# 1pathplanningzzj/pointnet_refine

Hardware: AMD Instinct MI355X
Metric: lane segments/sec (fwd+bwd) at B=4096,N=1024; HBM GB/s vs roofline (higher is better)
Workload: dtype f32 (large GEMMs: 2xfp16-split MFMA, 3 products, fp32 accumulate); 1 GPU; LineRefineNet training step (fwd + deep-supervision L1 + bwd + Adam), B=4096/GPU, N=1024, M=32, C=4; global_batch=4096, points=1024, parallelism=dp1, decoder_chunk=4096

## Files before the change

include/pointnet_refine_hip.h:

```cpp
#ifndef POINTNET_REFINE_HIP_H
#define POINTNET_REFINE_HIP_H

#include <stddef.h>
#include <stdint.h>

#ifdef __cplusplus
extern "C" {
#endif

#define PRH_OK 0
#define PRH_ERR_ARG (-1)
#define PRH_ERR_WORKSPACE (-2)
#define PRH_ERR_HIP (-3)

#define PRH_MAX_LAYERS 8

typedef struct {
  const float* w;
  const float* b;
  const float* gamma;
  const float* beta;
  float* running_mean;
  float* running_var;
  int64_t* num_batches_tracked;
// ... 17 lines not shown
  const float* gate_w2;
  const float* gate_b2;
} prh_encoder_params;

typedef struct {
  prh_bn_layer_grad conv[5];
  prh_bn_layer_grad fusion;
  float* d_gate_w1; float* d_gate_b1; float* d_gate_w2; float* d_gate_b2;
} prh_encoder_grads;

typedef struct {
  float* z_cat;
  float* z_fus;
  float* gate;
  float* bn_scale;
  float* bn_shift;
  float* bn_mean;
  float* bn_rstd;
  int32_t* argmax;
  float* op_amax;
} prh_encoder_saved;

size_t prh_encoder_workspace_bytes(int B, int N, int in_channel, int out_dim, int backward);

int prh_encoder_forward(const prh_encoder_params* prm, const float* ctx, int B, int N,
                        int training, float momentum, float eps,
                        float* fused, float* gfeat, const prh_encoder_saved* saved,
                        void* workspace, size_t workspace_bytes, int device, void* stream);

int prh_encoder_backward(const prh_encoder_params* prm, const float* ctx, int B, int N,
                         int training, float* d_fused, const float* d_gfeat, int d_fused_scratch,
                         const prh_encoder_saved* saved, const prh_encoder_grads* grads,
                         float* d_ctx, void* workspace, size_t workspace_bytes, int device,
                         void* stream);

typedef struct {
  uint16_t* z_cat;
  uint16_t* z_fus;
  uint16_t* gate;
  float* bn_scale;
  float* bn_shift;
  float* bn_mean;
  float* bn_rstd;
  int32_t* argmax;
} prh_encoder_saved_bf16;
size_t prh_encoder_bf16_workspace_bytes(int B, int N, int in_channel, int out_dim, int backward);
// ... 178 lines not shown
```

pointnet_refine_amd/_lib.py:

```python
from __future__ import annotations

import ctypes as C
import os
import subprocess
import threading

_HERE = os.path.dirname(os.path.abspath(__file__))
_ROOT = os.path.dirname(_HERE)
LIB_PATH = os.environ.get("PRH_LIB_PATH") or os.path.join(_HERE, "libpointnet_refine_hip.so")
_CSRC = os.path.join(_HERE, "csrc")
_SOURCES = [os.path.join(_CSRC, "prh_lib.hip")] + (sorted(
    os.path.join(_CSRC, f) for f in os.listdir(_CSRC) if f.endswith((".hpp", ".h", ".hip")) and f != "prh_lib.hip")
    if os.path.isdir(_CSRC) else [])
_HEADER = os.path.join(_ROOT, "include", "pointnet_refine_hip.h")

PRH_MAX_LAYERS = 8


class BnLayer(C.Structure):
    _fields_ = [("w", C.c_void_p), ("b", C.c_void_p), ("gamma", C.c_void_p), ("beta", C.c_void_p),
                ("running_mean", C.c_void_p), ("running_var", C.c_void_p),
                ("num_batches_tracked", C.c_void_p), ("cin", C.c_int), ("cout", C.c_int)]


# ... 5 lines not shown
    _fields_ = [("in_channel", C.c_int), ("out_dim", C.c_int), ("conv", BnLayer * 5),
                ("fusion", BnLayer), ("gate_w1", C.c_void_p), ("gate_b1", C.c_void_p),
                ("gate_w2", C.c_void_p), ("gate_b2", C.c_void_p)]


class EncoderGrads(C.Structure):
    _fields_ = [("conv", BnLayerGrad * 5), ("fusion", BnLayerGrad), ("d_gate_w1", C.c_void_p),
                ("d_gate_b1", C.c_void_p), ("d_gate_w2", C.c_void_p), ("d_gate_b2", C.c_void_p)]


class EncoderSaved(C.Structure):
    _fields_ = [("z_cat", C.c_void_p), ("z_fus", C.c_void_p), ("gate", C.c_void_p),
                ("bn_scale", C.c_void_p), ("bn_shift", C.c_void_p), ("bn_mean", C.c_void_p),
                ("bn_rstd", C.c_void_p), ("argmax", C.c_void_p), ("op_amax", C.c_void_p)]


class EncoderSavedBf16(C.Structure):
    _fields_ = [("z_cat", C.c_void_p), ("z_fus", C.c_void_p), ("gate", C.c_void_p),
                ("bn_scale", C.c_void_p), ("bn_shift", C.c_void_p), ("bn_mean", C.c_void_p),
                ("bn_rstd", C.c_void_p), ("argmax", C.c_void_p)]


EXPORTS = [
    "prh_encoder_workspace_bytes", "prh_encoder_forward", "prh_encoder_backward",
    "prh_encoder_bf16_workspace_bytes", "prh_encoder_forward_bf16", "prh_encoder_backward_bf16",
    "prh_linear_bf16_workspace_bytes", "prh_linear_forward_bf16", "prh_linear_backward_bf16",
    "prh_linear_forward_out16", "prh_linear_backward_dy16", "prh_attn_forward_kv16", "prh_attn_backward_kv16",
    "prh_encoder_fused_image_bytes", "prh_encoder_fused_prepare", "prh_encoder_fused_workspace_bytes",
    "prh_encoder_fused_forward",
    "prh_linear_forward_workspace_bytes", "prh_linear_forward", "prh_linear_forward_ex",
    "prh_linear_forward_full", "prh_operand_absmax_workspace_bytes", "prh_operand_absmax",
    "prh_linear_uses_operand_maxima", "prh_linear_backward_full", "prh_pos_hidden_forward", "prh_pos_hidden_backward_workspace_bytes",
    "prh_pos_hidden_backward", "prh_linear_small_forward", "prh_linear_small_backward_workspace_bytes",
    "prh_linear_small_backward",
    "prh_linear_backward_workspace_bytes", "prh_linear_backward", "prh_linear_backward_ex",
    "prh_mlp_stack_workspace_bytes", "prh_mlp_stack_forward", "prh_mlp_stack_backward",
    "prh_test_gemm_nt", "prh_test_gemm_tn_workspace_bytes", "prh_test_gemm_tn", "prh_test_xcc_map",
    "prh_profile_enable", "prh_profile_count", "prh_profile_reset", "prh_profile_read",
    "prh_attn_forward", "prh_attn_backward", "prh_attn_backward_ex",
    "prh_context_workspace_bytes", "prh_context_build",
    "prh_line_metrics", "prh_shift_sweep_workspace_bytes", "prh_shift_sweep",
    "prh_l1_loss_workspace_bytes", "prh_l1_loss", "prh_adam_step",
    "prh_add_dropout_layernorm_forward", "prh_add_dropout_layernorm_workspace_bytes",
    "prh_add_dropout_layernorm_backward",
    "prh_relu_mask_absmax", "prh_cast_perm_bf16", "prh_posmem_images", "prh_attn_fold_forward", "prh_set_gemm_mode", "prh_get_gemm_mode", "prh_set_dropout_seed_source",
    "prh_last_error", "prh_version",
]
# ... 7 lines not shown
        return True
    t = os.path.getmtime(LIB_PATH)
    return any(os.path.exists(s) and os.path.getmtime(s) > t for s in _SOURCES + [_HEADER])


def build(force: bool = False, verbose: bool = False) -> str:
    if not force and not needs_build():
        return LIB_PATH
    hipcc = os.environ.get("HIPCC", "/opt/rocm/bin/hipcc")
    cmd = [hipcc, "--offload-arch=gfx950", "-O3", "-std=c++17", "-shared", "-fPIC",
           "-o", LIB_PATH, _SOURCES[0]]
    if verbose:
        print(" ".join(cmd))
    subprocess.run(cmd, check=True)
    return LIB_PATH


def _bind(lib):
    vp, i, f, sz, lg = C.c_void_p, C.c_int, C.c_float, C.c_size_t, C.c_long
    lib.prh_last_error.restype = C.c_char_p
    lib.prh_version.restype = C.c_char_p
    lib.prh_encoder_workspace_bytes.restype = sz
    lib.prh_encoder_workspace_bytes.argtypes = [i, i, i, i, i]
    lib.prh_encoder_forward.restype = i
    lib.prh_encoder_forward.argtypes = [C.POINTER(EncoderParams), vp, i, i, i, f, f, vp, vp,
                                        C.POINTER(EncoderSaved), vp, sz, i, vp]
    lib.prh_encoder_backward.restype = i
    lib.prh_encoder_backward.argtypes = [C.POINTER(EncoderParams), vp, i, i, i, vp, vp, i,
                                         C.POINTER(EncoderSaved), C.POINTER(EncoderGrads), vp, vp,
                                         sz, i, vp]
    lib.prh_encoder_bf16_workspace_bytes.restype = sz
    lib.prh_encoder_bf16_workspace_bytes.argtypes = [i, i, i, i, i]
    lib.prh_encoder_forward_bf16.restype = i
    lib.prh_encoder_forward_bf16.argtypes = [C.POINTER(EncoderParams), vp, i, i, i, f, f, vp, vp,
                                             C.POINTER(EncoderSavedBf16), vp, sz, i, vp]
    lib.prh_encoder_backward_bf16.restype = i
    lib.prh_encoder_backward_bf16.argtypes = [C.POINTER(EncoderParams), vp, i, i, i, vp, vp,
                                              C.POINTER(EncoderSavedBf16), C.POINTER(EncoderGrads), vp, vp,
                                              sz, i, vp]
    lib.prh_linear_bf16_workspace_bytes.restype = sz
    lib.prh_linear_bf16_workspace_bytes.argtypes = [i, i, i, i]
    lib.prh_linear_forward_bf16.restype = i
    lib.prh_linear_forward_bf16.argtypes = [vp, lg, vp, vp, vp, i, i, i, i, vp, sz, i, vp]
    lib.prh_linear_backward_bf16.restype = i
    lib.prh_linear_backward_bf16.argtypes = [vp, lg, vp, vp, vp, vp, vp, i, i, i, vp, sz, i, vp]
    lib.prh_linear_forward_out16.restype = i
# ... 141 lines not shown
```

pointnet_refine_amd/csrc/prh_gemm.hpp:

```cpp
#pragma once
#include <hip/hip_runtime.h>
#include <type_traits>
#include <stdint.h>

namespace prh {

typedef float f32x16 __attribute__((ext_vector_type(16)));

enum { PRO_NONE = 0, PRO_BNRELU = 1, PRO_BNBWD = 2, PRO_GATE1 = 3 };
enum { EPI_BIAS = 0, EPI_BIAS_STATS = 1, EPI_GATE = 2, EPI_DGRAD = 3 };

enum {
  F_RELU_OUT = 1,
  F_ACCUM = 2,
  F_MASK = 4,
  F_STATS = 8,
  F_STORE_GATE = 16,
  F_E1_ROWVEC = 32,
  F_RESID = 64,
  F_DROPOUT = 256,
  F_POOL = 128,
};

struct NTParams {
// ... 41 lines not shown

__device__ __forceinline__ int lds_off(int row, int slot) {
  return row * BK + ((slot ^ ((row >> 1) & 7)) << 2);
}

template <int PRO>
__device__ __forceinline__ float4 pro_apply(float4 a, float4 a2, float4 ka, float4 kb, float4 kc) {
  float4 o;
  if (PRO == PRO_NONE) {
    o = a;
  } else if (PRO == PRO_BNRELU) {
    o.x = fmaxf(fmaf(a.x, ka.x, kb.x), 0.f); o.y = fmaxf(fmaf(a.y, ka.y, kb.y), 0.f);
    o.z = fmaxf(fmaf(a.z, ka.z, kb.z), 0.f); o.w = fmaxf(fmaf(a.w, ka.w, kb.w), 0.f);
  } else if (PRO == PRO_BNBWD) {
    o.x = fmaf(ka.x, a.x, fmaf(kb.x, a2.x, kc.x)); o.y = fmaf(ka.y, a.y, fmaf(kb.y, a2.y, kc.y));
    o.z = fmaf(ka.z, a.z, fmaf(kb.z, a2.z, kc.z)); o.w = fmaf(ka.w, a.w, fmaf(kb.w, a2.w, kc.w));
  } else {
    o.x = fmaxf(fmaf(a.x, ka.x, kb.x), 0.f); o.y = fmaxf(fmaf(a.x, ka.y, kb.y), 0.f);
    o.z = fmaxf(fmaf(a.x, ka.z, kb.z), 0.f); o.w = fmaxf(fmaf(a.x, ka.w, kb.w), 0.f);
  }
  return o;
}

__device__ __forceinline__ float4 ldg4(const float* p) { return *reinterpret_cast<const float4*>(p); }
__device__ __forceinline__ float4 zero4() { return make_float4(0.f, 0.f, 0.f, 0.f); }

template <int EPI, int MT, int NT>
__device__ __forceinline__ void nt_epilogue(f32x16 (&acc)[MT][NT], const NTParams& p, int rbase_,
                                            int cbase, int rb, int lane) {
  const int half = lane >> 5, l31 = lane & 31;
  const int rbase = __builtin_amdgcn_readfirstlane(rbase_);
  float* __restrict__ Cb = p.C + (size_t)rbase * p.ldc;
  const float* __restrict__ Eb = p.E1 != nullptr ? p.E1 + (size_t)rbase * p.lde1 : nullptr;
  float* __restrict__ C2b = p.C2 != nullptr ? p.C2 + (size_t)rbase * p.ldc2 : nullptr;
  const int ldc = (int)p.ldc, lde1 = (int)p.lde1, ldc2 = (int)p.ldc2;
  const int mrows = p.M - rbase;
  const unsigned dseed = (EPI == EPI_BIAS && (p.flags & F_DROPOUT) != 0) ? epi_seed(p) : 0u;
#pragma unroll
  for (int nt = 0; nt < NT; ++nt) {
    const int col = cbase + nt * 32 + l31;
    const bool cok = col < p.N;
    const float bias = (p.bias != nullptr && cok) ? p.bias[col] : 0.f;

    if (EPI == EPI_BIAS || EPI == EPI_BIAS_STATS) {
      float s = 0.f;
#pragma unroll
// ... 34 lines not shown
          float mx = -3.0e38f, mn = 3.0e38f;
#pragma unroll
          for (int mt = 0; mt < MT; ++mt)
#pragma unroll
            for (int r = 0; r < 16; ++r)
              if (mt * 32 + crow(r, half) < mrows) { mx = fmaxf(mx, acc[mt][nt][r]); mn = fminf(mn, acc[mt][nt][r]); }
          mx = fmaxf(mx, __shfl_xor(mx, 32));
          mn = fminf(mn, __shfl_xor(mn, 32));
          if (half == 0 && cok) {
            p.ws_c[(size_t)rb * p.N + col] = mx;
            p.ws_d[(size_t)rb * p.N + col] = mn;
          }
        }
      }
    } else if (EPI == EPI_GATE) {
      const float es = cok ? p.es[col] : 0.f, et = cok ? p.et[col] : 0.f;
#pragma unroll
      for (int mt = 0; mt < MT; ++mt)
#pragma unroll
        for (int r = 0; r < 16; ++r) {
          const int lr = mt * 32 + crow(r, half);
          if (lr < mrows && cok) {
            const float g = acc[mt][nt][r] + bias;
            const float m = 0.5f + 0.5f / (1.f + __expf(-g));
            const float zf = Eb[lr * lde1 + col];
            const float rl = fmaxf(fmaf(zf, es, et), 0.f);
            Cb[lr * ldc + col] = rl * m;
            if ((p.flags & F_STORE_GATE) != 0) C2b[lr * ldc2 + col] = m;
          }
        }
    } else {
      const bool mask = (p.flags & F_MASK) != 0, accum = (p.flags & F_ACCUM) != 0;
      const bool need_z = mask || (p.flags & F_STATS) != 0;
      const int ecol = (p.flags & F_E1_ROWVEC) ? 0 : col;
      const float es = (mask && cok) ? p.es[col] : 0.f, et = (mask && cok) ? p.et[col] : 0.f;
      float s1 = 0.f, s2 = 0.f;
#pragma unroll
      for (int mt = 0; mt < MT; ++mt)
#pragma unroll
        for (int r = 0; r < 16; ++r) {
          const int lr = mt * 32 + crow(r, half);
          if (lr < mrows && cok) {
            float v = acc[mt][nt][r] + bias;
            if (accum) v += Cb[lr * ldc + col];
            float z = 0.f;
            if (need_z) z = Eb[lr * lde1 + ecol];
            if (mask && !(fmaf(z, es, et) > 0.f)) v = 0.f;
// ... 261 lines not shown
      const int lr = mt * 32 + lrow;
      const bool ok = lr < mrows && c4ok;
      float4 v = *reinterpret_cast<const float4*>(scratch + lrow * EPI_LDW + c4);
      v.x += bias4.x; v.y += bias4.y; v.z += bias4.z; v.w += bias4.w;
      const float4 z = zz[b & 1][i];
      const float4 o = oo[b & 1][i];
      if (EPI == EPI_DGRAD) {
        v.x += o.x; v.y += o.y; v.z += o.z; v.w += o.w;
        if (mask) {
          v.x = fmaf(z.x, es4.x, et4.x) > 0.f ? v.x : 0.f;
          v.y = fmaf(z.y, es4.y, et4.y) > 0.f ? v.y : 0.f;
          v.z = fmaf(z.z, es4.z, et4.z) > 0.f ? v.z : 0.f;
          v.w = fmaf(z.w, es4.w, et4.w) > 0.f ? v.w : 0.f;
        }
        if (C16) {
          v.x = bf16_round(v.x); v.y = bf16_round(v.y); v.z = bf16_round(v.z); v.w = bf16_round(v.w);
        }
        const float4 q = ok ? v : zero4();
        s1.x += q.x; s1.y += q.y; s1.z += q.z; s1.w += q.w;
        s2.x = fmaf(q.x, z.x, s2.x); s2.y = fmaf(q.y, z.y, s2.y);
        s2.z = fmaf(q.z, z.z, s2.z); s2.w = fmaf(q.w, z.w, s2.w);
      } else if (EPI == EPI_GATE) {
        float4 m;
        m.x = 0.5f + 0.5f / (1.f + __expf(-v.x)); m.y = 0.5f + 0.5f / (1.f + __expf(-v.y));
        m.z = 0.5f + 0.5f / (1.f + __expf(-v.z)); m.w = 0.5f + 0.5f / (1.f + __expf(-v.w));
        v.x = fmaxf(fmaf(z.x, es4.x, et4.x), 0.f) * m.x; v.y = fmaxf(fmaf(z.y, es4.y, et4.y), 0.f) * m.y;
        v.z = fmaxf(fmaf(z.z, es4.z, et4.z), 0.f) * m.z; v.w = fmaxf(fmaf(z.w, es4.w, et4.w), 0.f) * m.w;
        if (ok && (p.flags & F_STORE_GATE) != 0) st4e<C16>(C2b, lr * ldc2 + col4, m);
        if (pool && ok) {
          if (C16) { v.x = bf16_round(v.x); v.y = bf16_round(v.y); v.z = bf16_round(v.z); v.w = bf16_round(v.w); }
          const float vv[4] = {v.x, v.y, v.z, v.w};
#pragma unroll
          for (int e = 0; e < 4; ++e) {
            if (vv[e] > pmx[e]) { pmx[e] = vv[e]; pix[e] = lr; }
            psm[e] += vv[e];
          }
        }
      } else {
        if (resid) { v.x += z.x; v.y += z.y; v.z += z.z; v.w += z.w; }
        if ((p.flags & F_RELU_OUT) != 0) {
          v.x = fmaxf(v.x, 0.f); v.y = fmaxf(v.y, 0.f); v.z = fmaxf(v.z, 0.f); v.w = fmaxf(v.w, 0.f);
        }
        if (EPI == EPI_BIAS && (p.flags & F_DROPOUT) != 0) {
          const unsigned rw = (unsigned)(rbase + lr), c0 = (unsigned)col4;
          v.x = epi_keep(dseed, rw, c0, p.drop_thresh) ? v.x * p.drop_scale : 0.f;
          v.y = epi_keep(dseed, rw, c0 + 1, p.drop_thresh) ? v.y * p.drop_scale : 0.f;
          v.z = epi_keep(dseed, rw, c0 + 2, p.drop_thresh) ? v.z * p.drop_scale : 0.f;
          v.w = epi_keep(dseed, rw, c0 + 3, p.drop_thresh) ? v.w * p.drop_scale : 0.f;
// ... 147 lines not shown
      if (it == 0) epi_block_to_scratch(acc, mt, scratch, lane);
      const int lrow = it * 4 + rr;
      const int lr = mt * 32 + lrow;
      const bool ok = lr < mrows && c4ok;
      float4 v = *reinterpret_cast<const float4*>(scratch + lrow * EPI_LDW + c4);
      v.x += bias4.x; v.y += bias4.y; v.z += bias4.z; v.w += bias4.w;
      const float4 z = ev_f4(zz[b & 1][i]);
      const float4 o = ev_f4(oo[b & 1][i]);
      if (EPI == EPI_DGRAD) {
        v.x += o.x; v.y += o.y; v.z += o.z; v.w += o.w;
        v.x = fmaf(z.x, es4.x, et4.x) > mthr ? v.x : 0.f;
        v.y = fmaf(z.y, es4.y, et4.y) > mthr ? v.y : 0.f;
        v.z = fmaf(z.z, es4.z, et4.z) > mthr ? v.z : 0.f;
        v.w = fmaf(z.w, es4.w, et4.w) > mthr ? v.w : 0.f;
        if (C16) {
          v.x = bf16_round(v.x); v.y = bf16_round(v.y); v.z = bf16_round(v.z); v.w = bf16_round(v.w);
        }
        const float4 q = ok ? v : zero4();
        s1.x += q.x; s1.y += q.y; s1.z += q.z; s1.w += q.w;
        s2.x = fmaf(q.x, z.x, s2.x); s2.y = fmaf(q.y, z.y, s2.y);
        s2.z = fmaf(q.z, z.z, s2.z); s2.w = fmaf(q.w, z.w, s2.w);
      } else if (EPI == EPI_GATE) {
        float4 m;
        m.x = 0.5f + 0.5f / (1.f + __expf(-v.x)); m.y = 0.5f + 0.5f / (1.f + __expf(-v.y));
        m.z = 0.5f + 0.5f / (1.f + __expf(-v.z)); m.w = 0.5f + 0.5f / (1.f + __expf(-v.w));
        v.x = fmaxf(fmaf(z.x, es4.x, et4.x), 0.f) * m.x; v.y = fmaxf(fmaf(z.y, es4.y, et4.y), 0.f) * m.y;
        v.z = fmaxf(fmaf(z.z, es4.z, et4.z), 0.f) * m.z; v.w = fmaxf(fmaf(z.w, es4.w, et4.w), 0.f) * m.w;
        if ((p.flags & F_STORE_GATE) != 0) ev_store(rsC2, lr * rowC2 + vC, m);
        if (pool && ok) {
          if (C16) { v.x = bf16_round(v.x); v.y = bf16_round(v.y); v.z = bf16_round(v.z); v.w = bf16_round(v.w); }
          const float vv[4] = {v.x, v.y, v.z, v.w};
#pragma unroll
          for (int e = 0; e < 4; ++e) {
            if (vv[e] > pmx[e]) { pmx[e] = vv[e]; pix[e] = lr; }
            psm[e] += vv[e];
          }
        }
      } else {
        if (resid) { v.x += z.x; v.y += z.y; v.z += z.z; v.w += z.w; }
        if ((p.flags & F_RELU_OUT) != 0) {
          v.x = fmaxf(v.x, 0.f); v.y = fmaxf(v.y, 0.f); v.z = fmaxf(v.z, 0.f); v.w = fmaxf(v.w, 0.f);
        }
        if (EPI == EPI_BIAS && (p.flags & F_DROPOUT) != 0) {
          const unsigned rw = (unsigned)(rbase + lr), c0 = (unsigned)col4;
          v.x = epi_keep(dseed, rw, c0, p.drop_thresh) ? v.x * p.drop_scale : 0.f;
          v.y = epi_keep(dseed, rw, c0 + 1, p.drop_thresh) ? v.y * p.drop_scale : 0.f;
          v.z = epi_keep(dseed, rw, c0 + 2, p.drop_thresh) ? v.z * p.drop_scale : 0.f;
          v.w = epi_keep(dseed, rw, c0 + 3, p.drop_thresh) ? v.w * p.drop_scale : 0.f;
// ... 282 lines not shown
```

pointnet_refine_amd/csrc/prh_gemm_h2.hpp:

```cpp
#pragma once
#include "prh_gemm_s3.hpp"

namespace prh {

constexpr int H2_BK = 32;
constexpr int H2_PLANE = 256 * H2_BK * 2;
constexpr int H2_OPER = 2 * H2_PLANE;
constexpr int H2_STAGE = 2 * H2_OPER;
constexpr int H2_LDS = 2 * H2_STAGE;

__device__ __forceinline__ int h2_off(int row, int k) {
  return row * 64 + ((((k >> 3) ^ (-(row >> 2))) & 3) << 4) + ((k & 7) << 1);
}

inline size_t h2_weight_bytes(int N, int K) {
  return S3_WHDR + (size_t)((N + 255) / 256) * ((K + H2_BK - 1) / H2_BK) * H2_OPER;
}

__global__ __launch_bounds__(256) void prep_weights_h2_kernel(const float* __restrict__ W, int N,
                                                              int K, long ldw, char* __restrict__ out,
                                                              const float* __restrict__ amax) {
  const int KT = (K + H2_BK - 1) / H2_BK;
  const int NT_ = (N + 255) / 256;
  const long total = (long)NT_ * 256 * KT * 4;
// ... 2 lines not shown
  const int chunk = (int)(i & 3);
  long t = i >> 2;
  const int k_tile = (int)(t % KT); t /= KT;
  const int row = (int)(t & 255);
  const int n_tile = (int)(t >> 8);
  const int n = n_tile * 256 + row;
  const float S = pow2_scale(load_amax(amax));
  float v[8];
#pragma unroll
  for (int j = 0; j < 8; ++j) {
    const int k = k_tile * H2_BK + chunk * 8 + j;
    v[j] = (n < N && k < K) ? W[(size_t)n * ldw + k] * S : 0.f;
  }
  uint4 h, l;
  split2h(v[0], v[1], h.x, l.x);
  split2h(v[2], v[3], h.y, l.y);
  split2h(v[4], v[5], h.z, l.z);
  split2h(v[6], v[7], h.w, l.w);
  char* base = out + ((size_t)n_tile * KT + k_tile) * H2_OPER + h2_off(row, chunk * 8);
  *reinterpret_cast<uint4*>(base) = h;
  *reinterpret_cast<uint4*>(base + H2_PLANE) = l;
}

template <int I0 = 0, int I1 = 8>
__device__ __forceinline__ void h2_compute(f32x4 (&acc)[8][4], const char* st, int wm, int wn, int l15,
                                           int kc) {
  f16x8 wh[4], wl[4];
#pragma unroll
  for (int j = 0; j < 4; ++j) {
    const char* q = st + H2_OPER + h2_off(wn + j * 16 + l15, kc * 8);
    wh[j] = *reinterpret_cast<const f16x8*>(q);
    wl[j] = *reinterpret_cast<const f16x8*>(q + H2_PLANE);
  }
#pragma unroll
  for (int i = I0; i < I1; ++i) {
    const char* q = st + h2_off(wm + i * 16 + l15, kc * 8);
    const f16x8 ah = *reinterpret_cast<const f16x8*>(q);
    const f16x8 al = *reinterpret_cast<const f16x8*>(q + H2_PLANE);
#pragma unroll
    for (int j = 0; j < 4; ++j) {
      acc[i][j] = __builtin_amdgcn_mfma_f32_16x16x32_f16(al, wh[j], acc[i][j], 0, 0, 0);
      acc[i][j] = __builtin_amdgcn_mfma_f32_16x16x32_f16(ah, wl[j], acc[i][j], 0, 0, 0);
      acc[i][j] = __builtin_amdgcn_mfma_f32_16x16x32_f16(ah, wh[j], acc[i][j], 0, 0, 0);
    }
  }
}

template <int PRO, int EPI, bool PP = false>
__global__ __launch_bounds__(512, 2) void gemm_nt_h2_kernel(const NTParams p,
                                                            const char* __restrict__ Wp) {
  static_assert(PRO == PRO_NONE || PRO == PRO_BNRELU || PRO == PRO_GATE1, "prologue not supported");
  extern __shared__ __attribute__((aligned(16))) char smem[];
#ifdef PRH_STAMP
  unsigned t_acc[4] = {0u, 0u, 0u, 0u};
  unsigned long long t_prev = __builtin_amdgcn_s_memtime();
#endif
  const int tid = threadIdx.x, lane = tid & 63, wave = tid >> 6;
  const int l15 = lane & 15, kc = lane >> 4;
  const int wm = (wave >> 2) * 128, wn = (wave & 3) * 64;
  const int vb = xcd_remap(blockIdx.x, gridDim.x);
  const int tile_n = vb % p.tiles_n, tile_m = vb / p.tiles_n;
  const int m0 = tile_m * 256, n0 = tile_n * 256;
  const int KT = (p.K + H2_BK - 1) / H2_BK;

  const int sc = (tid & 7) * 4;
  const int sr = tid >> 3;
  const int KP = (KT + 2) * H2_BK;
// ... 438 lines not shown
```

pointnet_refine_amd/csrc/prh_lib.hip:

```cpp
#include "../../include/pointnet_refine_hip.h"

#include <hip/hip_runtime.h>
#include <stdarg.h>
#include <stdio.h>
#include <string.h>

#include <mutex>
#include <vector>

#include <stdlib.h>

#include "prh_gemm.hpp"
#include "prh_attn.hpp"
#include "prh_attn16.hpp"
#include "prh_gemm_s3.hpp"
#include "prh_gemm_h2.hpp"
#include "prh_b16.hpp"
#include "prh_small.hpp"
#include "prh_attnfold.hpp"
#include "prh_fused.hpp"
#include "prh_context.hpp"
#include "prh_metrics.hpp"
#include "prh_kernels.hpp"

// ... 1281 lines not shown
  LAUNCH_CHECK();
  StatInfo si; si.count = cdiv(P, 64); si.rows = 64;
  return stack_backward(c, layers, L, x, P, training, dy_cat, ldz, z_cat, ldz, bn_scale, bn_shift,
                        bn_mean, bn_rstd, grads, dx, w, sc, si, st);
}

static int enc_cat(const prh_encoder_params* prm) {
  int c = 0;
  for (int l = 0; l < 5; ++l) c += prm->conv[l].cout;
  return c;
}

size_t prh_encoder_workspace_bytes(int B, int N, int in_channel, int out_dim, int backward) {
  const int P = B * N;
  prh_bn_layer ly[5];
  const int ch[6] = {in_channel, 64, 128, 256, 512, out_dim};
  for (int l = 0; l < 5; ++l) { ly[l].cin = ch[l]; ly[l].cout = ch[l + 1]; }
  const int cat = 64 + 128 + 256 + 512 + out_dim;
  Arena a; EncWS e;
  enc_carve(cores_of(gemm_mode()), a, e, P, ly, cat, out_dim, backward);
  return a.off + 256;
}

static int check_encoder(const prh_encoder_params* prm) {
  if (!prm) return fail(PRH_ERR_ARG, "encoder: null params");
  if (prm->in_channel < 4) return fail(PRH_ERR_ARG, "encoder: expected input to have at least 4 channels (x,y,z,intensity), got %d", prm->in_channel);
  if (prm->conv[0].cin != prm->in_channel) return fail(PRH_ERR_ARG, "encoder: conv1.cin != in_channel");
  TRY(check_stack(prm->conv, 5));
  if (prm->conv[4].cout != prm->out_dim) return fail(PRH_ERR_ARG, "encoder: conv5.cout != out_dim");
  if (prm->fusion.cin != enc_cat(prm) || prm->fusion.cout != prm->out_dim)
    return fail(PRH_ERR_ARG, "encoder: fusion layer shape mismatch");
  if (prm->out_dim % 4) return fail(PRH_ERR_ARG, "encoder: out_dim must be a multiple of 4");
  if (!prm->fusion.w || !prm->fusion.b || !prm->fusion.gamma || !prm->fusion.beta ||
      !prm->fusion.running_mean || !prm->fusion.running_var || !prm->gate_w1 || !prm->gate_b1 ||
      !prm->gate_w2 || !prm->gate_b2)
    return fail(PRH_ERR_ARG, "encoder: null parameter pointer");
  return PRH_OK;
}

int prh_encoder_forward(const prh_encoder_params* prm, const float* ctx, int B, int N,
                        int training, float momentum, float eps, float* fused, float* gfeat,
                        const prh_encoder_saved* sv, void* workspace, size_t workspace_bytes,
                        int device, void* stream) {
  TRY(check_encoder(prm));
  if (!ctx || !fused || !sv || !sv->z_cat || !sv->z_fus || !sv->bn_scale || !sv->bn_shift ||
      !sv->bn_mean || !sv->bn_rstd || B <= 0 || N <= 0)
// ... 18 lines not shown
    NTParams p; memset(&p, 0, sizeof(p));
    p.A = sv->z_cat; p.lda = cat; p.W = prm->fusion.w; p.ldw = cat; p.K = cat;
    p.pa = sv->bn_scale; p.pb = sv->bn_shift;
    p.M = P; p.N = od; p.bias = prm->fusion.b; p.C = sv->z_fus; p.ldc = od;
    p.ws_a = w.ws_a; p.ws_b = w.ws_b; p.wprep = w.wprep;
    if (op_amax != nullptr) {
      hipLaunchKernelGGL(max_of_kernel, dim3(1), dim3(1), 0, st, (const float*)op_amax, 5, op_amax + 5);
      LAUNCH_CHECK();
      p.amaxA = op_amax + 5;
      p.ws_c = w.ws_c; p.ws_d = w.ws_d;
    }
    StatInfo si;
    if (training) TRY((launch_nt<PRO_BNRELU, EPI_BIAS_STATS>(c, p, st, &si)));
    else TRY((launch_nt<PRO_BNRELU, EPI_BIAS>(c, p, st)));
    TRY(bn_coeffs(prm->fusion, P, training, momentum, eps, w.ws_a, w.ws_b, w.stat2, si, sv->bn_mean + cat,
                  sv->bn_rstd + cat, sv->bn_scale + cat, sv->bn_shift + cat, st, w.ws_c, w.ws_d, w.apart,
                  op_amax ? op_amax + 6 : nullptr));
  }
  {
    NTParams p; memset(&p, 0, sizeof(p));
    p.A = ctx + 3; p.lda = C; p.pa = prm->gate_w1; p.pb = prm->gate_b1;
    p.W = prm->gate_w2; p.ldw = 64; p.K = 64; p.M = P; p.N = od; p.bias = prm->gate_b2;
    p.E1 = sv->z_fus; p.lde1 = od; p.es = sv->bn_scale + cat; p.et = sv->bn_shift + cat;
    p.C = fused; p.ldc = od; p.C2 = sv->gate; p.ldc2 = od;
    p.wprep = w.wprep;
    p.flags = sv->gate ? F_STORE_GATE : 0;
    const bool fuse_pool = gfeat != nullptr && (N % 128) == 0 && c.mode == 3 &&
                           nt_use_s3(c, P, od, 64) && (od & 3) == 0;
    if (fuse_pool) { p.flags |= F_POOL; p.ws_a = w.ws_a; p.ws_b = w.ws_b; p.ws_c = w.ws_c; }
    TRY((launch_nt<PRO_GATE1, EPI_GATE>(c, p, st)));
    if ((p.flags & F_POOL) != 0) {
      hipLaunchKernelGGL(pool_tiles_kernel, dim3(cdiv(od, 256), B), dim3(256), 0, st, (const float*)w.ws_a,
                         (const float*)w.ws_b, (const int*)w.ws_c, N / 128, N, od, gfeat, sv->argmax);
      LAUNCH_CHECK();
      return PRH_OK;
    }
  }
  if (gfeat != nullptr) {
    hipLaunchKernelGGL(pool_kernel, dim3(cdiv(od, 64), B), dim3(256), 0, st, fused, N, od, gfeat,
                       sv->argmax);
    LAUNCH_CHECK();
  }
  return PRH_OK;
}

int prh_encoder_backward(const prh_encoder_params* prm, const float* ctx, int B, int N,
                         int training, float* d_fused, const float* d_gfeat, int d_fused_scratch,
                         const prh_encoder_saved* sv, const prh_encoder_grads* gr, float* d_ctx,
                         void* workspace, size_t workspace_bytes, int device, void* stream) {
// ... 2 lines not shown
    return fail(PRH_ERR_ARG, "encoder_backward: bad argument (a gradient and saved.gate are required)");
  if (d_gfeat && !sv->argmax) return fail(PRH_ERR_ARG, "encoder_backward: d_gfeat needs saved.argmax");
  const int P = B * N;
  HIP_TRY(hipSetDevice(device));
  hipStream_t st = (hipStream_t)stream;
  const int cat = enc_cat(prm), od = prm->out_dim, C = prm->in_channel;
  const Cores c = cores_of(gemm_mode());
  Arena a(workspace, workspace_bytes);
  EncWS ews;
  if (d_fused_scratch && (d_fused == nullptr || d_gfeat != nullptr))
    return fail(PRH_ERR_ARG, "encoder_backward: d_fused_scratch needs d_fused and no d_gfeat");
  enc_carve(c, a, ews, P, prm->conv, cat, od, d_fused_scratch ? 2 : 1);
  StackWS& w = ews.w;
  StackBwdScratch& sc = ews.sc;
  float *fslab = ews.fslab, *fcslab = ews.fcslab, *dy_cat = ews.dy_cat, *dU = ews.dU, *dyf = d_fused_scratch ? d_fused : ews.dyf;
  float *gsum_a = ews.gsum_a, *gsum_b = ews.gsum_b;
  if (!a.ok) return fail(PRH_ERR_WORKSPACE, "encoder_backward: workspace too small (%zu bytes)", workspace_bytes);
  StackDims d = stack_dims(prm->conv, 5);
  if (d.cin0p != d.cin0) {
    TRY(copy_cols(ctx, d.cin0, d.cin0, w.xpad, d.cin0p, d.cin0p, (size_t)P, st));
    TRY(copy_cols(prm->conv[0].w, d.cin0, d.cin0, w.w0pad, d.cin0p, d.cin0p, (size_t)prm->conv[0].cout, st));
  }

  hipLaunchKernelGGL(combine_bwd_kernel, dim3(cdiv(P, 64), cdiv(od, 64)), dim3(256), 0, st, d_fused,
                     d_gfeat, sv->argmax, sv->z_fus, sv->gate, sv->bn_scale + cat,
                     sv->bn_shift + cat, P, N, od, dyf, w.ws_a, w.ws_b);
  LAUNCH_CHECK();
  hipLaunchKernelGGL(bn_stage1_kernel, dim3(cdiv(od, 32), BN_SLICES), dim3(256), 0, st, w.ws_a, w.ws_b,
                     cdiv(P, 64), (long)od, od, 64, P, 0, w.stat2);
  LAUNCH_CHECK();
  hipLaunchKernelGGL(bn_bwd_finalize_kernel, dim3(cdiv(od, 128)), dim3(128), 0, st, w.stat2, P, od,
                     prm->fusion.gamma, sv->bn_mean + cat, sv->bn_rstd + cat,
                     training, sc.ca, sc.cb, sc.cc, gr->fusion.dgamma, gr->fusion.dbeta,
                     gr->fusion.db);
  LAUNCH_CHECK();
  float* dG = sv->gate;

  StatInfo si5;
  const float* dzf_amax = nullptr;
  const bool matf = dz_in_place(c, od, (long)od, (long)od);
  if (matf) {
    TRY(materialize_dz(dyf, (long)od, sv->z_fus, (long)od, sc.ca, sc.cb, sc.cc, P, od, sc.hdr, st));
    dzf_amax = sc.hdr;
  }
  if (gr->fusion.dw) {
    TNParams t; memset(&t, 0, sizeof(t));
    t.A = dyf; t.lda = od; t.A2 = sv->z_fus; t.lda2 = od; t.pa = sc.ca; t.pb = sc.cb; t.pc = sc.cc;
    t.B = sv->z_cat; t.ldb = cat; t.qa = sv->bn_scale; t.qb = sv->bn_shift;
    t.P = P; t.Mo = od; t.Ni = cat;
// ... 939 lines not shown
```

pointnet_refine_amd/ops.py:

```python
from __future__ import annotations

import ctypes as C
import math
import threading
from typing import List, Optional, Sequence

import torch

from . import _lib as L

_workspaces = {}


def _ws(device: torch.device, nbytes: int) -> torch.Tensor:
    key = (device.index, torch.cuda.current_stream(device).cuda_stream)
    t = _workspaces.get(key)
    if t is None or t.numel() < nbytes:
        _workspaces.pop(key, None)
        t = None
        t = torch.empty(int(nbytes * 1.05) + 4096, dtype=torch.uint8, device=device)
        _workspaces[key] = t
    return t


# ... 609 lines not shown
        x = x.contiguous()
        B, N, Cin = x.shape
        p2 = list(params)
        for i in (0, 2, 4, 6, 8, 20, 24, 26):
            p2[i] = params[i].reshape(params[i].shape[0], -1).contiguous()
        for t in p2:
            _req_gpu_f32(t, "parameter")
        if Cin != p2[0].shape[1]:
            raise RuntimeError(f"Given groups=1, weight of size {list(params[0].shape)}, expected input"
                               f"[{B}, {Cin}, {N}] to have {p2[0].shape[1]} channels, but got {Cin} channels instead")
        if training and B * N < 2:
            raise ValueError(f"Expected more than 1 value per channel when training, got input size {(B, Cin, N)}")
        if training:
            invalidate_fused_images()
        out_dim = p2[8].shape[0]
        cat = 64 + 128 + 256 + 512 + out_dim
        P = B * N
        need_bwd = any(ctx.needs_input_grad)
        ctx.bf16 = L.lib().prh_get_gemm_mode() == 4
        if ctx.bf16:
            return EncoderFn._forward_bf16(ctx, x, want_global, training, momentum, eps, buffers, params, p2, need_bwd)
        z_cat = torch.empty((P, cat), dtype=torch.float32, device=dev)
        z_fus = torch.empty((P, out_dim), dtype=torch.float32, device=dev)
        gate = torch.empty((P, out_dim), dtype=torch.float32, device=dev) if need_bwd else None
        coef = torch.empty((5, cat + out_dim), dtype=torch.float32, device=dev)
        fused = torch.empty((B, N, out_dim), dtype=torch.float32, device=dev)
        gfeat = torch.empty((B, 2 * out_dim), dtype=torch.float32, device=dev) if want_global else None
        argmax = torch.empty((B, out_dim), dtype=torch.int32, device=dev) if (want_global and need_bwd) else None
        prm = _enc_params_struct(p2, buffers, Cin)
        gemm_mode = L.lib().prh_get_gemm_mode()
        sv = L.EncoderSaved(_p(z_cat), _p(z_fus), _p(gate), _p(coef[0]), _p(coef[1]), _p(coef[2]),
                            _p(coef[3]), _p(argmax), _p(coef[4]) if (training and need_bwd) else None)
        nb = L.lib().prh_encoder_workspace_bytes(B, N, Cin, out_dim, 0)
        ws = _ws(dev, nb)
        L.check(L.lib().prh_encoder_forward(C.byref(prm), _p(x), B, N, int(training), float(momentum),
                                            float(eps), _p(fused), _p(gfeat), C.byref(sv), _p(ws),
                                            ws.numel(), dev.index, _stream(dev)),
                "prh_encoder_forward")
        if need_bwd:
            ctx.save_for_backward(x, z_cat, z_fus, gate, coef, argmax if argmax is not None else coef, *p2)
            ctx.has_argmax = argmax is not None
            ctx.training = int(training)
            ctx.gemm_mode = gemm_mode
            ctx.pshapes = [t.shape for t in params]
            ctx.sinks = [_sink_view(t) for t in params]
            ctx.consumed = False
        ctx_amax = coef[4, 6:7] if (training and need_bwd and gemm_mode == 3) else None
        EncoderFn.last_fused_amax = ctx_amax
        if want_global:
            return gfeat, fused
        return None, fused

    @staticmethod
    def _forward_bf16(ctx, x, want_global, training, momentum, eps, buffers, params, p2, need_bwd):
        dev = x.device
        B, N, Cin = x.shape
        out_dim = p2[8].shape[0]
        cat = 64 + 128 + 256 + 512 + out_dim
        P = B * N
        bf = torch.bfloat16
        z_cat = torch.empty((P, cat), dtype=bf, device=dev)
        z_fus = torch.empty((P, out_dim), dtype=bf, device=dev)
        gate = torch.empty((P, out_dim), dtype=bf, device=dev) if need_bwd else None
        coef = torch.empty((4, cat + out_dim), dtype=torch.float32, device=dev)
        fused = torch.empty((B, N, out_dim), dtype=bf, device=dev)
        gfeat = torch.empty((B, 2 * out_dim), dtype=torch.float32, device=dev) if want_global else None
# ... 44 lines not shown
        gr.d_gate_w1, gr.d_gate_b1, gr.d_gate_w2, gr.d_gate_b2 = _p(g[24]), _p(g[25]), _p(g[26]), _p(g[27])
        dx = torch.empty_like(x) if ctx.needs_input_grad[0] else None
        nb = L.lib().prh_encoder_bf16_workspace_bytes(B, N, Cin, out_dim, 1)
        ws = _ws(dev, nb)
        L.check(L.lib().prh_encoder_backward_bf16(C.byref(prm), _p(x), B, N, ctx.training, _p(d_fused), _p(d_gfeat),
                                                  C.byref(sv), C.byref(gr), _p(dx), _p(ws), ws.numel(), dev.index,
                                                  _stream(dev)), "prh_encoder_backward_bf16")
        grads = [_grad_ret(*b_) for b_ in gb]
        grads = [gi.reshape(s) if gi is not None else None for gi, s in zip(grads, ctx.pshapes)]
        return (dx, None, None, None, None, None, *grads)

    @staticmethod
    def backward(ctx, d_gfeat, d_fused):
        if ctx.consumed:
            raise RuntimeError("pointnet_refine_amd encoder: backward through the same graph a second "
                               "time is not supported by default (the saved gate buffer, 4 KB per point, is "
                               "overwritten by its gradient); call ops.allow_encoder_retain_graph(True) before "
                               "the first backward to work on a copy instead")
        ctx.consumed = not ENCODER_RETAIN_GRAPH
        if ctx.bf16:
            return EncoderFn._backward_bf16(ctx, d_gfeat, d_fused)
        saved = ctx.saved_tensors
        x, z_cat, z_fus, gate, coef, argmax = saved[:6]
        if ENCODER_RETAIN_GRAPH:
            gate = gate.clone()
        p2 = list(saved[6:])
        dev = x.device
        B, N, Cin = x.shape
        out_dim = p2[8].shape[0]
        scratch = (d_fused is not None and d_gfeat is None and d_fused.is_contiguous() and not ENCODER_RETAIN_GRAPH
                   and d_fused.dtype == torch.float32
                   and (d_fused._base is None or d_fused._base.numel() == d_fused.numel()))
        if d_fused is not None:
            d_fused = d_fused.contiguous()
        if d_gfeat is not None:
            if not ctx.has_argmax:
                raise RuntimeError("encoder backward: gradient for global_feat but no argmax saved")
            d_gfeat = d_gfeat.contiguous()
        prm = _enc_params_struct(p2, None, Cin)
        same_mode = ctx.training and ctx.gemm_mode == L.lib().prh_get_gemm_mode()
        sv = L.EncoderSaved(_p(z_cat), _p(z_fus), _p(gate), _p(coef[0]), _p(coef[1]), _p(coef[2]),
                            _p(coef[3]), _p(argmax) if ctx.has_argmax else None,
                            _p(coef[4]) if same_mode else None)
        gb = [_grad_buf(ctx.sinks[i], t.shape, dev) for i, t in enumerate(p2)]
        g = [b_[0] for b_ in gb]
        gr = L.EncoderGrads()
        for k in range(5):
            gr.conv[k] = L.BnLayerGrad(_p(g[2 * k]), _p(g[2 * k + 1]), _p(g[10 + 2 * k]), _p(g[11 + 2 * k]))
        gr.fusion = L.BnLayerGrad(_p(g[20]), _p(g[21]), _p(g[22]), _p(g[23]))
        gr.d_gate_w1, gr.d_gate_b1, gr.d_gate_w2, gr.d_gate_b2 = _p(g[24]), _p(g[25]), _p(g[26]), _p(g[27])
        dx = torch.empty_like(x) if ctx.needs_input_grad[0] else None
        nb = L.lib().prh_encoder_workspace_bytes(B, N, Cin, out_dim, 2 if scratch else 1)
# ... 498 lines not shown
```

Baseline: 9513 segments/s.

## Recompute encoder gate in backward instead of storing it in forward

In the 2xfp16-split GEMM mode, the forward no longer writes the P x out_dim fp32 gate tensor. The backward instead rebuilds it inside a new fused combine kernel, which redoes the small gate MLP (K=64) with split-fp16 MFMA from the intensity channel and gate weights. This saves one large HBM write in forward and replaces a large read in backward with a small GEMM recompute, plus two absmax passes to recover the scaling. The trade-off is extra compute, and the backward's dG output still goes into a freshly allocated buffer.

```diff
diff --git a/include/pointnet_refine_hip.h b/include/pointnet_refine_hip.h
--- a/include/pointnet_refine_hip.h
+++ b/include/pointnet_refine_hip.h
@@ -63,6 +63,8 @@
 } prh_encoder_saved;
 
 size_t prh_encoder_workspace_bytes(int B, int N, int in_channel, int out_dim, int backward);
+
+int prh_encoder_recomputes_gate(int B, int N, int out_dim);
 
 int prh_encoder_forward(const prh_encoder_params* prm, const float* ctx, int B, int N,
                         int training, float momentum, float eps,
diff --git a/pointnet_refine_amd/_lib.py b/pointnet_refine_amd/_lib.py
--- a/pointnet_refine_amd/_lib.py
+++ b/pointnet_refine_amd/_lib.py
@@ -51,7 +51,7 @@
 
 
 EXPORTS = [
-    "prh_encoder_workspace_bytes", "prh_encoder_forward", "prh_encoder_backward",
+    "prh_encoder_workspace_bytes", "prh_encoder_forward", "prh_encoder_backward", "prh_encoder_recomputes_gate",
     "prh_encoder_bf16_workspace_bytes", "prh_encoder_forward_bf16", "prh_encoder_backward_bf16",
     "prh_linear_bf16_workspace_bytes", "prh_linear_forward_bf16", "prh_linear_backward_bf16",
     "prh_linear_forward_out16", "prh_linear_backward_dy16", "prh_attn_forward_kv16", "prh_attn_backward_kv16",
@@ -105,6 +105,8 @@
     lib.prh_version.restype = C.c_char_p
     lib.prh_encoder_workspace_bytes.restype = sz
     lib.prh_encoder_workspace_bytes.argtypes = [i, i, i, i, i]
+    lib.prh_encoder_recomputes_gate.restype = i
+    lib.prh_encoder_recomputes_gate.argtypes = [i, i, i]
     lib.prh_encoder_forward.restype = i
     lib.prh_encoder_forward.argtypes = [C.POINTER(EncoderParams), vp, i, i, i, f, f, vp, vp,
                                         C.POINTER(EncoderSaved), vp, sz, i, vp]
diff --git a/pointnet_refine_amd/csrc/prh_gemm.hpp b/pointnet_refine_amd/csrc/prh_gemm.hpp
--- a/pointnet_refine_amd/csrc/prh_gemm.hpp
+++ b/pointnet_refine_amd/csrc/prh_gemm.hpp
@@ -87,6 +87,8 @@
   return o;
 }
 
+__device__ __forceinline__ float gate_of(float g) { return 0.5f + 0.5f / (1.f + __expf(-g)); }
+
 __device__ __forceinline__ float4 ldg4(const float* p) { return *reinterpret_cast<const float4*>(p); }
 __device__ __forceinline__ float4 zero4() { return make_float4(0.f, 0.f, 0.f, 0.f); }
 
@@ -167,7 +169,7 @@
           const int lr = mt * 32 + crow(r, half);
           if (lr < mrows && cok) {
             const float g = acc[mt][nt][r] + bias;
-            const float m = 0.5f + 0.5f / (1.f + __expf(-g));
+            const float m = gate_of(g);
             const float zf = Eb[lr * lde1 + col];
             const float rl = fmaxf(fmaf(zf, es, et), 0.f);
             Cb[lr * ldc + col] = rl * m;
@@ -475,8 +477,7 @@
         s2.z = fmaf(q.z, z.z, s2.z); s2.w = fmaf(q.w, z.w, s2.w);
       } else if (EPI == EPI_GATE) {
         float4 m;
-        m.x = 0.5f + 0.5f / (1.f + __expf(-v.x)); m.y = 0.5f + 0.5f / (1.f + __expf(-v.y));
-        m.z = 0.5f + 0.5f / (1.f + __expf(-v.z)); m.w = 0.5f + 0.5f / (1.f + __expf(-v.w));
+        m.x = gate_of(v.x); m.y = gate_of(v.y); m.z = gate_of(v.z); m.w = gate_of(v.w);
         v.x = fmaxf(fmaf(z.x, es4.x, et4.x), 0.f) * m.x; v.y = fmaxf(fmaf(z.y, es4.y, et4.y), 0.f) * m.y;
         v.z = fmaxf(fmaf(z.z, es4.z, et4.z), 0.f) * m.z; v.w = fmaxf(fmaf(z.w, es4.w, et4.w), 0.f) * m.w;
         if (ok && (p.flags & F_STORE_GATE) != 0) st4e<C16>(C2b, lr * ldc2 + col4, m);
@@ -670,8 +671,7 @@
         s2.z = fmaf(q.z, z.z, s2.z); s2.w = fmaf(q.w, z.w, s2.w);
       } else if (EPI == EPI_GATE) {
         float4 m;
-        m.x = 0.5f + 0.5f / (1.f + __expf(-v.x)); m.y = 0.5f + 0.5f / (1.f + __expf(-v.y));
-        m.z = 0.5f + 0.5f / (1.f + __expf(-v.z)); m.w = 0.5f + 0.5f / (1.f + __expf(-v.w));
+        m.x = gate_of(v.x); m.y = gate_of(v.y); m.z = gate_of(v.z); m.w = gate_of(v.w);
         v.x = fmaxf(fmaf(z.x, es4.x, et4.x), 0.f) * m.x; v.y = fmaxf(fmaf(z.y, es4.y, et4.y), 0.f) * m.y;
         v.z = fmaxf(fmaf(z.z, es4.z, et4.z), 0.f) * m.z; v.w = fmaxf(fmaf(z.w, es4.w, et4.w), 0.f) * m.w;
         if ((p.flags & F_STORE_GATE) != 0) ev_store(rsC2, lr * rowC2 + vC, m);
diff --git a/pointnet_refine_amd/csrc/prh_gemm_h2.hpp b/pointnet_refine_amd/csrc/prh_gemm_h2.hpp
--- a/pointnet_refine_amd/csrc/prh_gemm_h2.hpp
+++ b/pointnet_refine_amd/csrc/prh_gemm_h2.hpp
@@ -48,6 +48,12 @@
   *reinterpret_cast<uint4*>(base + H2_PLANE) = l;
 }
 
+__device__ __forceinline__ f32x4 h2_mac3(f16x8 ah, f16x8 al, f16x8 wh, f16x8 wl, f32x4 acc) {
+  acc = __builtin_amdgcn_mfma_f32_16x16x32_f16(al, wh, acc, 0, 0, 0);
+  acc = __builtin_amdgcn_mfma_f32_16x16x32_f16(ah, wl, acc, 0, 0, 0);
+  return __builtin_amdgcn_mfma_f32_16x16x32_f16(ah, wh, acc, 0, 0, 0);
+}
+
 template <int I0 = 0, int I1 = 8>
 __device__ __forceinline__ void h2_compute(f32x4 (&acc)[8][4], const char* st, int wm, int wn, int l15,
                                            int kc) {
@@ -64,11 +70,136 @@
     const f16x8 ah = *reinterpret_cast<const f16x8*>(q);
     const f16x8 al = *reinterpret_cast<const f16x8*>(q + H2_PLANE);
 #pragma unroll
-    for (int j = 0; j < 4; ++j) {
-      acc[i][j] = __builtin_amdgcn_mfma_f32_16x16x32_f16(al, wh[j], acc[i][j], 0, 0, 0);
-      acc[i][j] = __builtin_amdgcn_mfma_f32_16x16x32_f16(ah, wl[j], acc[i][j], 0, 0, 0);
-      acc[i][j] = __builtin_amdgcn_mfma_f32_16x16x32_f16(ah, wh[j], acc[i][j], 0, 0, 0);
-    }
+    for (int j = 0; j < 4; ++j) acc[i][j] = h2_mac3(ah, al, wh[j], wl[j], acc[i][j]);
+  }
+}
+
+__device__ __forceinline__ void h2_gate1_fragment(float gi, const float* __restrict__ w1, const float* __restrict__ b1,
+                                                  float sA, int k0, f16x8& h, f16x8& l) {
+  uint4 hh, ll;
+  unsigned* ph = &hh.x;
+  unsigned* pl = &ll.x;
+#pragma unroll
+  for (int q = 0; q < 2; ++q) {
+    const int k = k0 + 4 * q;
+    const float4 ka = make_float4(w1[k] * sA, w1[k + 1] * sA, w1[k + 2] * sA, w1[k + 3] * sA);
+    const float4 kb = make_float4(b1[k] * sA, b1[k + 1] * sA, b1[k + 2] * sA, b1[k + 3] * sA);
+    const float4 v = pro_apply<PRO_GATE1>(make_float4(gi, 0.f, 0.f, 0.f), zero4(), ka, kb, zero4());
+    split2h(v.x, v.y, ph[2 * q], pl[2 * q]);
+    split2h(v.z, v.w, ph[2 * q + 1], pl[2 * q + 1]);
+  }
+  h = __builtin_bit_cast(f16x8, hh);
+  l = __builtin_bit_cast(f16x8, ll);
+}
+
+__device__ __forceinline__ void h2_weight_fragment(const float* __restrict__ W, int N, int K, long ldw, float S,
+                                                   int n, int k0, f16x8& h, f16x8& l) {
+  float v[8];
+#pragma unroll
+  for (int j = 0; j < 8; ++j) {
+    const int k = k0 + j;
+    v[j] = (n < N && k < K) ? W[(size_t)n * ldw + k] * S : 0.f;
+  }
+  uint4 hh, ll;
+  split2h(v[0], v[1], hh.x, ll.x);
+  split2h(v[2], v[3], hh.y, ll.y);
+  split2h(v[4], v[5], hh.z, ll.z);
+  split2h(v[6], v[7], hh.w, ll.w);
+  h = __builtin_bit_cast(f16x8, hh);
+  l = __builtin_bit_cast(f16x8, ll);
+}
+
+__device__ __forceinline__ float unscale_add(float a, float u, float b) {
+#pragma clang fp contract(off)
+  return a * u + b;
+}
+
+__global__ __launch_bounds__(256) void gate_combine_bwd_kernel(
+    const float* dF, const float* __restrict__ d_gfeat, const int32_t* __restrict__ argmax,
+    const float* __restrict__ zf, const float* __restrict__ inten, long ldi, const float* __restrict__ w1,
+    const float* __restrict__ b1, const float* __restrict__ W2, const float* __restrict__ b2,
+    const float* __restrict__ amax, const float* __restrict__ s, const float* __restrict__ t, int P, int N,
+    int C, float* dy_out, float* dG, float* ws_a, float* ws_b) {
+  __shared__ float sm[64][65];
+  __shared__ float r1[4][64], r2[4][64];
+  const int tid = threadIdx.x, lane = tid & 63, wave = tid >> 6;
+  const int l15 = lane & 15, kc = lane >> 4;
+  const int cbase = blockIdx.x * 64;
+  const float sA = pow2_scale(load_amax(amax + 1));
+  const float sW = pow2_scale(load_amax(amax));
+  const float unscale = 1.f / (sA * sW);
+  f16x8 wh[4][2], wl[4][2];
+  float bias[4];
+#pragma unroll
+  for (int j = 0; j < 4; ++j) {
+    const int col = cbase + j * 16 + l15;
+#pragma unroll
+    for (int kt = 0; kt < 2; ++kt) h2_weight_fragment(W2, C, 64, 64, sW, col, kt * H2_BK + kc * 8, wh[j][kt], wl[j][kt]);
+    bias[j] = col < C ? b2[col] : 0.f;
+  }
+  const int c = tid & 63, g = tid >> 6;
+  const int col = cbase + c;
+  const float sc = col < C ? s[col] : 0.f, sh = col < C ? t[col] : 0.f;
+  const int tiles = (P + 63) / 64;
+  for (int tile = blockIdx.y; tile < tiles; tile += gridDim.y) {
+    const int rbase = tile * 64;
+    const int row0 = rbase + g * 16;
+    float dv[16], zv[16];
+#pragma unroll
+    for (int i = 0; i < 16; ++i) {
+      const bool ok = col < C && row0 + i < P;
+      const size_t off = (size_t)(row0 + i) * C + col;
+      dv[i] = (ok && dF != nullptr) ? dF[off] : 0.f;
+      zv[i] = ok ? zf[off] : 0.f;
+    }
+    {
+      const int row = rbase + wave * 16 + l15;
+      const float gi = row < P ? inten[(size_t)row * ldi] : 0.f;
+      f16x8 ah[2], al[2];
+#pragma unroll
+      for (int kt = 0; kt < 2; ++kt) h2_gate1_fragment(gi, w1, b1, sA, kt * H2_BK + kc * 8, ah[kt], al[kt]);
+#pragma unroll
+      for (int j = 0; j < 4; ++j) {
+        f32x4 acc = {0.f, 0.f, 0.f, 0.f};
+#pragma unroll
+        for (int kt = 0; kt < 2; ++kt) acc = h2_mac3(ah[kt], al[kt], wh[j][kt], wl[j][kt], acc);
+#pragma unroll
+        for (int r = 0; r < 4; ++r) sm[wave * 16 + kc * 4 + r][j * 16 + l15] = gate_of(unscale_add(acc[r], unscale, bias[j]));
+      }
+    }
+    __syncthreads();
+    float s1 = 0.f, s2 = 0.f;
+    if (col < C) {
+#pragma unroll
+      for (int i = 0; i < 16; ++i) {
+        const int row = row0 + i;
+        if (row >= P) break;
+        const size_t off = (size_t)row * C + col;
+        float d = dv[i];
+        if (d_gfeat != nullptr) {
+          const int b = row / N, n = row - b * N;
+          d += d_gfeat[(size_t)b * 2 * C + C + col] / (float)N;
+          if (argmax[(size_t)b * C + col] == n) d += d_gfeat[(size_t)b * 2 * C + col];
+        }
+        const float z = zv[i], m = sm[g * 16 + i][c];
+        const float pre = fmaf(z, sc, sh);
+        const float r = fmaxf(pre, 0.f);
+        const float sig = 2.f * m - 1.f;
+        const float dy = pre > 0.f ? d * m : 0.f;
+        dG[off] = d * r * 0.5f * sig * (1.f - sig);
+        dy_out[off] = dy;
+        s1 += dy;
+        s2 = fmaf(dy, z, s2);
+      }
+    }
+    r1[g][c] = s1; r2[g][c] = s2;
+    __syncthreads();
+    if (g == 0 && col < C) {
+      for (int j = 1; j < 4; ++j) { s1 += r1[j][c]; s2 += r2[j][c]; }
+      ws_a[(size_t)tile * C + col] = s1;
+      ws_b[(size_t)tile * C + col] = s2;
+    }
+    __syncthreads();
   }
 }
 
diff --git a/pointnet_refine_amd/csrc/prh_lib.hip b/pointnet_refine_amd/csrc/prh_lib.hip
--- a/pointnet_refine_amd/csrc/prh_lib.hip
+++ b/pointnet_refine_amd/csrc/prh_lib.hip
@@ -1327,6 +1327,13 @@
   return a.off + 256;
 }
 
+inline bool gate_recomputed(Cores c, int P, int od) { return c.mode == 3 && c.core == 3 && nt_use_s3(c, P, od, 64); }
+
+int prh_encoder_recomputes_gate(int B, int N, int out_dim) {
+  if (B <= 0 || N <= 0 || (long)B * N > 2000000000L || out_dim % 4) return 0;
+  return gate_recomputed(cores_of(gemm_mode()), B * N, out_dim) ? 1 : 0;
+}
+
 static int check_encoder(const prh_encoder_params* prm) {
   if (!prm) return fail(PRH_ERR_ARG, "encoder: null params");
   if (prm->in_channel < 4) return fail(PRH_ERR_ARG, "encoder: expected input to have at least 4 channels (x,y,z,intensity), got %d", prm->in_channel);
@@ -1391,9 +1398,10 @@
     p.A = ctx + 3; p.lda = C; p.pa = prm->gate_w1; p.pb = prm->gate_b1;
     p.W = prm->gate_w2; p.ldw = 64; p.K = 64; p.M = P; p.N = od; p.bias = prm->gate_b2;
     p.E1 = sv->z_fus; p.lde1 = od; p.es = sv->bn_scale + cat; p.et = sv->bn_shift + cat;
-    p.C = fused; p.ldc = od; p.C2 = sv->gate; p.ldc2 = od;
+    const bool store_gate = sv->gate != nullptr && !gate_recomputed(c, P, od);
+    p.C = fused; p.ldc = od; p.C2 = store_gate ? sv->gate : nullptr; p.ldc2 = od;
     p.wprep = w.wprep;
-    p.flags = sv->gate ? F_STORE_GATE : 0;
+    p.flags = store_gate ? F_STORE_GATE : 0;
     const bool fuse_pool = gfeat != nullptr && (N % 128) == 0 && c.mode == 3 &&
                            nt_use_s3(c, P, od, 64) && (od & 3) == 0;
     if (fuse_pool) { p.flags |= F_POOL; p.ws_a = w.ws_a; p.ws_b = w.ws_b; p.ws_c = w.ws_c; }
@@ -1442,9 +1450,22 @@
     TRY(copy_cols(prm->conv[0].w, d.cin0, d.cin0, w.w0pad, d.cin0p, d.cin0p, (size_t)prm->conv[0].cout, st));
   }
 
-  hipLaunchKernelGGL(combine_bwd_kernel, dim3(cdiv(P, 64), cdiv(od, 64)), dim3(256), 0, st, d_fused,
-                     d_gfeat, sv->argmax, sv->z_fus, sv->gate, sv->bn_scale + cat,
-                     sv->bn_shift + cat, P, N, od, dyf, w.ws_a, w.ws_b);
+  if (gate_recomputed(c, P, od)) {
+    float* hdr = reinterpret_cast<float*>(w.wprep);
+    TRY((measure_absmax<PRO_NONE>(prm->gate_w2, 64, nullptr, 0, nullptr, nullptr, nullptr, od, 64, hdr, hdr + 64, st)));
+    TRY((measure_absmax<PRO_GATE1>(ctx + 3, C, nullptr, 0, prm->gate_w1, prm->gate_b1, nullptr, P, 64, hdr + 1,
+                                   hdr + 64, st)));
+    int slices = (int)cdiv(2048, cdiv(od, 64));
+    slices = slices > (int)cdiv(P, 64) ? (int)cdiv(P, 64) : slices;
+    hipLaunchKernelGGL(gate_combine_bwd_kernel, dim3(cdiv(od, 64), slices), dim3(256), 0, st, d_fused,
+                       d_gfeat, sv->argmax, sv->z_fus, ctx + 3, (long)C, prm->gate_w1, prm->gate_b1,
+                       prm->gate_w2, prm->gate_b2, (const float*)hdr, sv->bn_scale + cat, sv->bn_shift + cat,
+                       P, N, od, dyf, sv->gate, w.ws_a, w.ws_b);
+  } else {
+    hipLaunchKernelGGL(combine_bwd_kernel, dim3(cdiv(P, 64), cdiv(od, 64)), dim3(256), 0, st, d_fused,
+                       d_gfeat, sv->argmax, sv->z_fus, sv->gate, sv->bn_scale + cat,
+                       sv->bn_shift + cat, P, N, od, dyf, w.ws_a, w.ws_b);
+  }
   LAUNCH_CHECK();
   hipLaunchKernelGGL(bn_stage1_kernel, dim3(cdiv(od, 32), BN_SLICES), dim3(256), 0, st, w.ws_a, w.ws_b,
                      cdiv(P, 64), (long)od, od, 64, P, 0, w.stat2);
diff --git a/pointnet_refine_amd/ops.py b/pointnet_refine_amd/ops.py
--- a/pointnet_refine_amd/ops.py
+++ b/pointnet_refine_amd/ops.py
@@ -655,13 +655,14 @@
             return EncoderFn._forward_bf16(ctx, x, want_global, training, momentum, eps, buffers, params, p2, need_bwd)
         z_cat = torch.empty((P, cat), dtype=torch.float32, device=dev)
         z_fus = torch.empty((P, out_dim), dtype=torch.float32, device=dev)
-        gate = torch.empty((P, out_dim), dtype=torch.float32, device=dev) if need_bwd else None
+        gemm_mode = L.lib().prh_get_gemm_mode()
+        recompute = bool(L.lib().prh_encoder_recomputes_gate(B, N, out_dim))
+        gate = torch.empty((P, out_dim), dtype=torch.float32, device=dev) if (need_bwd and not recompute) else None
         coef = torch.empty((5, cat + out_dim), dtype=torch.float32, device=dev)
         fused = torch.empty((B, N, out_dim), dtype=torch.float32, device=dev)
         gfeat = torch.empty((B, 2 * out_dim), dtype=torch.float32, device=dev) if want_global else None
         argmax = torch.empty((B, out_dim), dtype=torch.int32, device=dev) if (want_global and need_bwd) else None
         prm = _enc_params_struct(p2, buffers, Cin)
-        gemm_mode = L.lib().prh_get_gemm_mode()
         sv = L.EncoderSaved(_p(z_cat), _p(z_fus), _p(gate), _p(coef[0]), _p(coef[1]), _p(coef[2]),
                             _p(coef[3]), _p(argmax), _p(coef[4]) if (training and need_bwd) else None)
         nb = L.lib().prh_encoder_workspace_bytes(B, N, Cin, out_dim, 0)
@@ -675,6 +676,7 @@
             ctx.has_argmax = argmax is not None
             ctx.training = int(training)
             ctx.gemm_mode = gemm_mode
+            ctx.gate_recomputed = recompute
             ctx.pshapes = [t.shape for t in params]
             ctx.sinks = [_sink_view(t) for t in params]
             ctx.consumed = False
@@ -765,12 +767,17 @@
             return EncoderFn._backward_bf16(ctx, d_gfeat, d_fused)
         saved = ctx.saved_tensors
         x, z_cat, z_fus, gate, coef, argmax = saved[:6]
-        if ENCODER_RETAIN_GRAPH:
-            gate = gate.clone()
         p2 = list(saved[6:])
         dev = x.device
         B, N, Cin = x.shape
         out_dim = p2[8].shape[0]
+        if ctx.gate_recomputed:
+            if not L.lib().prh_encoder_recomputes_gate(B, N, out_dim):
+                raise RuntimeError("pointnet_refine_amd encoder: the forward left the gate to be recomputed, which the "
+                                   "current GEMM mode does not do; run the backward in the forward's GEMM mode")
+            gate = torch.empty((B * N, out_dim), dtype=torch.float32, device=dev)
+        elif ENCODER_RETAIN_GRAPH:
+            gate = gate.clone()
         scratch = (d_fused is not None and d_gfeat is None and d_fused.is_contiguous() and not ENCODER_RETAIN_GRAPH
                    and d_fused.dtype == torch.float32
                    and (d_fused._base is None or d_fused._base.numel() == d_fused.numel()))
```

After: 9617 segments/s, median of 6. 1.1% higher.
